# Merricx/zksnake

Measured on AMD Instinct MI355X. Metric: BN254 G1 MSM throughput, higher is better.
Workload: dtype u32 limbs (254-bit modular integers)

## Files before the change

zksnake_amd/csrc/msm_impl.hip.h:

```cpp
#pragma once
#include <algorithm>
#include <chrono>
#include <memory>
#include <vector>
#include "common.hip.h"
#include "msm_plan.h"
#include "pair.hip.h"
#include "setup_impl.hip.h"
#include "codec.hip.h"
#include "glv_params.h"

#include "msm_common.hip.h"
#include "msm_accumulate.hip.h"
#include "msm_reduce.hip.h"

namespace zkmi {
using mem::DevBuf;

#if defined(ZK_GROUP) && (!defined(ZK_PART) || ZK_PART == 0)
extern template __global__ void accumulate_kernel<ZK_GROUP>(const uint32_t*, const uint32_t*, const uint32_t*, const uint32_t*, uint32_t, uint32_t, uint32_t, uint32_t*, uint32_t*);
extern template __global__ void accumulate_split_kernel<ZK_GROUP>(const uint32_t*, const uint32_t*, const uint32_t*, const uint32_t*, uint32_t, uint32_t, uint32_t, uint32_t*, uint32_t*);
extern template __global__ void bases_to_mont_kernel<ZK_GROUP>(const uint32_t*, uint64_t, uint32_t*, int);
extern template __global__ void combine_kernel<ZK_GROUP>(const uint32_t*, const uint32_t*, uint32_t, uint32_t, const uint32_t*, const uint32_t*, uint32_t*);
extern template __global__ void strided_sum_kernel<ZK_GROUP>(const uint32_t*, uint32_t*, SumJob, SumJob, uint32_t);
extern template __global__ void weighted_sum_kernel<ZK_GROUP>(const uint32_t*, uint32_t, uint32_t, const uint32_t*, uint32_t, uint32_t*);
ZK_SETUP_EXTERN_TEMPLATES(ZK_GROUP)
ZK_CODEC_EXTERN_TEMPLATES(ZK_GROUP)
#endif

#if !defined(ZK_PART) || ZK_PART == 0

template <class G>
static int precompute_table(uint32_t* table, uint64_t n, int c, int w_first, int w_count) {
    typedef typename G::F F;
    constexpr int AW = 2 * F::LIMBS, XW = 4 * F::LIMBS;
    if (w_first == 0 && w_count == 1) return ZK_OK;
    DevBuf temp_buf;
    ZK_HIP_RC(temp_buf.alloc(n * XW * 4));
    uint32_t* const temp = temp_buf.as();
    const unsigned blocks = (unsigned)((n + 255) / 256);
    const unsigned nblocks = (unsigned)((n + (uint64_t)NORM_THREADS * NORM_E - 1) / ((uint64_t)NORM_THREADS * NORM_E));
    hipLaunchKernelGGL(dbl_rows_kernel<G>, dim3(blocks), dim3(256), 0, 0, temp, n, c * w_first, (const uint32_t*)table);
    if (w_first > 0) hipLaunchKernelGGL(normalize_kernel<G>, dim3(nblocks), dim3(NORM_THREADS), 0, 0, temp, n, table, 0);
    for (int k = 1; k < w_count; ++k) {
        hipLaunchKernelGGL(dbl_rows_kernel<G>, dim3(blocks), dim3(256), 0, 0, temp, n, c, (const uint32_t*)nullptr);
        hipLaunchKernelGGL(normalize_kernel<G>, dim3(nblocks), dim3(NORM_THREADS), 0, 0, temp, n, table + (size_t)k * n * AW, 0);
    }
    ZK_HIP(hipGetLastError());
    ZK_HIP(hipDeviceSynchronize());
    return ZK_OK;
}

template <class G>
struct FixedTable {
    std::vector<uint64_t> base;
    DevBuf d_table;
    int nwin = 0;
    std::mutex mu;
    static FixedTable& get() {
        static FixedTable* const t = new FixedTable();
        return *t;
    }
    void release() {
        std::lock_guard<std::mutex> lock(mu);
        d_table.reset();
        base.clear();
    }
    int ensure(const uint64_t* base_limbs) {
        typedef typename G::F F;
        typedef typename G::Fr FrP;
        constexpr int AW = 2 * F::LIMBS, XW = 4 * F::LIMBS;
        const size_t words64 = AW / 2;
        if (d_table && base.size() == words64 && memcmp(base.data(), base_limbs, words64 * 8) == 0) return ZK_OK;
        d_table.reset();
        base.clear();
        nwin = (FrP::BITS + 1 + FIXED_C - 1) / FIXED_C;
        std::vector<uint32_t> wb((size_t)nwin * AW);
        {
            const uint32_t* w = reinterpret_cast<const uint32_t*>(base_limbs);
            Affine<F> g = {F::from_canonical(w), F::from_canonical(w + F::LIMBS)};
            XYZZ<F> acc = xyzz_from_affine<F>(g);
            for (int j = 0; j < nwin; ++j) {
                Affine<F> a = xyzz_to_affine<F>(acc);
                F::store(wb.data() + (size_t)j * AW, a.x);
                F::store(wb.data() + (size_t)j * AW + F::LIMBS, a.y);
                if (j + 1 < nwin) for (int k = 0; k < FIXED_C; ++k) acc = xyzz_dbl<F>(acc);
            }
        }
        const uint64_t rows = (uint64_t)nwin * FIXED_HALF;
        DevBuf table, d_wb, temp;
        ZK_HIP_RC(table.alloc(rows * AW * 4));
        ZK_HIP_RC(d_wb.alloc(wb.size() * 4));
        ZK_HIP_RC(temp.alloc(rows * XW * 4));
        ZK_HIP(hipMemcpy(d_wb.as(), wb.data(), wb.size() * 4, hipMemcpyHostToDevice));
        hipLaunchKernelGGL(fixed_table_kernel<G>, dim3((unsigned)((rows + 255) / 256)), dim3(256), 0, 0, d_wb.as(), nwin, temp.as());
        hipLaunchKernelGGL(normalize_kernel<G>, dim3((unsigned)((rows + (uint64_t)NORM_THREADS * NORM_E - 1) / ((uint64_t)NORM_THREADS * NORM_E))),
                           dim3(NORM_THREADS), 0, 0, temp.as(), rows, table.as(), 0);
        ZK_HIP(hipGetLastError());
        ZK_HIP(hipDeviceSynchronize());
        d_table = std::move(table);
        base.assign(base_limbs, base_limbs + words64);
        return ZK_OK;
    }
};

template <class G>
struct MsmPlan : MsmPlanBase {
    typedef typename G::F F;
    typedef typename G::Fr FrP;
    static constexpr int AW = 2 * F::LIMBS;
    static constexpr int XW = 4 * F::LIMBS;
    static constexpr uint64_t SEG_TARGET_LANES = 256ull * 1024;
    static constexpr int MAX_C = 20;
    bool wide = false;

    struct Work {
        DevBuf partials, buckets, rows, fin;
        DevBuf parts;
        hipEvent_t ev_acc0 = nullptr, ev_accs = nullptr, ev_acc1 = nullptr;
        bool acc_from_accs = false;
        hipEvent_t ev_release = nullptr;
        bool lent = false;
        uint32_t seg_len = 0;
        int w_first = 0, w_count = 0;
        uint32_t groups = 0;
    };

    uint64_t n = 0;
    uint64_t n_api = 0;
    bool glv = false;
    bool pre = false;
    int pw_first = 0, pw_count = 0;
    uint32_t B = 0, R = 0, C = 0;
    uint32_t bpr = 0, bpc = 0;
    Work ws;
    MsmFront front;
    std::shared_ptr<DevBuf> bases_block;
    uint32_t* d_bases = nullptr;
    uint32_t* h_final = nullptr;
    hipEvent_t ev_start = nullptr, ev_end = nullptr;

    ~MsmPlan() override {
        (void)hipDeviceSynchronize();
        pinned_free_cached(h_final);
        for (hipEvent_t e : {ws.ev_acc0, ws.ev_accs, ws.ev_acc1, ws.ev_release, ev_start, ev_end}) if (e) (void)hipEventDestroy(e);
        stream_release((create_flags & ZK_MSM_HIGH_PRIORITY) != 0, own_stream);
    }

    int init(uint64_t n_points, const void* bases, int bases_on_device, int flags, int window_bits, int win_first, int win_count,
             const MsmPlan* share = nullptr) {
        const bool trace = opt.trace_init;
        auto t_prev = std::chrono::steady_clock::now();
        auto mark = [&](const char* what) {
            if (!trace) return;
            auto now = std::chrono::steady_clock::now();
            fprintf(stderr, "[plan init] %-24s %8.1f us\n", what, std::chrono::duration<double, std::micro>(now - t_prev).count());
            t_prev = now;
        };
        create_flags = flags;
        seg_lanes_at_init = opt.segment_lanes ? opt.segment_lanes : SEG_TARGET_LANES;
        pre = (flags & ZK_MSM_PRECOMPUTE) != 0;
        if (n_points == 0 || n_points > (1ull << 26)) return fail(ZK_ERR_ARG, "MSM size must be in [1, 2^26]");
        const MsmLayout lay = msm_layout(FrP::BITS, GlvOf<G>::OK, n_points, flags, window_bits, win_count <= 0);
        glv = share ? share->glv : lay.glv;
        n_api = n_points;
        n = glv ? 2 * n_points : n_points;
        entries_per_window = n;
        c = lay.c;
        if (c < 2 || c > MAX_C) return fail(ZK_ERR_ARG, "window bits must be in [2, 20]");
        if (c > 16 && !pre) return fail(ZK_ERR_ARG, "windows wider than 16 bits need a fixed-base plan (ZK_MSM_PRECOMPUTE)");
        wide = c > 16;
        nwin = glv ? glv_window_count(c) : window_count(FrP::BITS + 1, c);
        if (win_count <= 0) { win_first = 0; win_count = nwin; }
        if (win_first < 0 || win_first + win_count > nwin) return fail(ZK_ERR_ARG, "window range out of bounds");
        pw_first = win_first;
        pw_count = win_count;
        B = 1u << (c - 1);
        int rl = (c - 1 + 1) / 2;
        if (rl > 8 && !wide) rl = 8;
        R = 1u << rl;
        C = B / R;
        if (C > 1024 || R > 1024) return fail(ZK_ERR_ARG, "window too wide for the reduction stage");
        bpr = (R + WS_BLOCK - 1) / WS_BLOCK;
        bpc = (C + WS_BLOCK - 1) / WS_BLOCK;
        const uint64_t entries = (uint64_t)pw_count * n;
        if (entries > 0x7FFFFFFFull) return fail(ZK_ERR_ARG, "MSM too large");

        ZK_HIP_RC(stream_acquire((flags & ZK_MSM_HIGH_PRIORITY) != 0, &own_stream));
        if (share) {
            bases_block = share->bases_block;
            d_bases = share->d_bases;
        } else {
            bases_block = std::make_shared<DevBuf>();
            ZK_HIP_RC(bases_block->alloc((pre ? (uint64_t)pw_count : 1ull) * n * AW * 4));
            d_bases = bases_block->as();
            if (bases_on_device) {
                hipLaunchKernelGGL(bases_to_mont_kernel<G>, dim3((unsigned)((n_api + 127) / 128)), dim3(128), 0, 0,
                                   (const uint32_t*)bases, n_api, d_bases, glv ? 1 : 0);
            } else {
                DevBuf tmp;
                ZK_HIP_RC(tmp.alloc(n_api * AW * 4));
                ZK_HIP(hipMemcpy(tmp.as(), bases, n_api * AW * 4, hipMemcpyHostToDevice));
                hipLaunchKernelGGL(bases_to_mont_kernel<G>, dim3((unsigned)((n_api + 127) / 128)), dim3(128), 0, 0, tmp.as(), n_api, d_bases, glv ? 1 : 0);
                ZK_HIP(hipDeviceSynchronize());
            }
            ZK_HIP(hipGetLastError());
            if (pre) {
                int rc = precompute_table<G>(d_bases, n, c, pw_first, pw_count);
                if (rc) return rc;
            }
        }
        mark("stream + bases");
        {
            FrontLayout fl;
            fl.c = c; fl.B = B; fl.n = n; fl.n_api = n_api; fl.pre = pre; fl.wide = wide; fl.glv = glv ? &GlvOf<G>::P::K : nullptr;
            fl.pw_first = pw_first; fl.pw_count = pw_count; fl.nwin = nwin; fl.curve = G::CURVE;
            ZK_HIP_RC(front.init(fl, &opt));
        }
        const uint64_t max_sets = pre ? 1ull : (uint64_t)pw_count;
        ZK_HIP_RC(pinned_alloc_cached((void**)&h_final, (size_t)max_sets * (bpr + bpc) * 2 * XW * 4));
        mark("scalars/digits/pinned");
        ZK_HIP(hipEventCreateWithFlags(&ev_start, hipEventDisableSystemFence));
        ZK_HIP(hipEventCreate(&ev_end));
        {
            const uint64_t keys = max_sets * B;
            const uint32_t seg_full = pick_seg_len(entries);
            const uint64_t max_segs = std::max<uint64_t>(entries / seg_full, std::min<uint64_t>(entries / 8, seg_lanes_at_init)) + keys + 8;
            ZK_HIP_RC(front.alloc_workspace());
            ZK_HIP_RC(ws.partials.alloc(max_segs * XW * 4));
            ZK_HIP_RC(ws.buckets.alloc(keys * XW * 4));
            ZK_HIP_RC(ws.rows.alloc(max_sets * (R + C) * XW * 4));
            if (sum_part_len() >= 2) ZK_HIP_RC(ws.parts.alloc(max_sets * 2 * (uint64_t)(B / sum_part_len()) * XW * 4));
            ZK_HIP_RC(ws.fin.alloc(max_sets * (bpr + bpc) * 2 * XW * 4));
            for (hipEvent_t* e : {&ws.ev_acc0, &ws.ev_accs, &ws.ev_acc1, &ws.ev_release}) ZK_HIP(hipEventCreate(e));
        }
        mark("workspace + events");
        ZK_HIP_RC(front.set_kernel_attributes());
        ZK_HIP(hipFuncSetAttribute((const void*)weighted_sum_kernel<G>, hipFuncAttributeMaxDynamicSharedMemorySize,
                                   (int)(HalfRegs<F>::COUNT * HS_THREADS * 4)));
        mark("func attributes");
        ZK_HIP(hipDeviceSynchronize());
        mark("device sync");
        return ZK_OK;
    }

    uint32_t sum_part_len() const {
        const uint32_t k = 16u;
        return (R >= 4 * k && C >= 4 * k) ? k : 0u;
    }

    uint32_t pick_seg_len(uint64_t entries) const {
        const uint64_t target = opt.segment_lanes ? opt.segment_lanes : SEG_TARGET_LANES;
        uint64_t sl = (entries + target - 1) / target;
        if (sl < 8) sl = 8;
        if (sl > 64) sl = 64;
        if (pre) {
            uint64_t per_bucket = entries / B;
            uint64_t want = (per_bucket + 11) / 12;
            if (want > sl) sl = want;
            if (sl > 1024) sl = 1024;
        }
        return (uint32_t)sl;
    }


    int stage_accumulate(uint32_t m, const SortedView& sv, hipStream_t st, bool prio_steps) {
        Work& l = ws;
        uint32_t *const partials = l.partials.as(), *const buckets = l.buckets.as();
        const uint32_t seg_len = sv.seg_len;
        const uint32_t n_keys = l.groups * B;
        const uint64_t lanes_needed = ((uint64_t)l.w_count * m + seg_len - 1) / seg_len;
        bool launched = false;
        if constexpr (AccumulateSplit<G>::ON) {
            if (opt.split_pairs < 0 ? AccumulateSplit<G>::DEFAULT : opt.split_pairs != 0) {
                hipLaunchKernelGGL(accumulate_split_kernel<G>, dim3((unsigned)((2 * lanes_needed + 255) / 256)), dim3(256), 0, st, d_bases, sv.sorted, sv.bstart, sv.sstart, n_keys, seg_len, prio_steps ? 1u : 0u, partials, buckets);
                launched = true;
            }
        }
        if (!launched) hipLaunchKernelGGL(accumulate_kernel<G>, dim3((unsigned)((lanes_needed + 255) / 256)), dim3(256), 0, st, d_bases, sv.sorted, sv.bstart, sv.sstart, n_keys, seg_len, prio_steps ? 1u : 0u, partials, buckets);
        ZK_HIP(hipEventRecord(l.ev_acc1, st));
        const uint32_t small_blocks = (2 * n_keys + COMBINE_THREADS - 1) / COMBINE_THREADS;
        hipLaunchKernelGGL(combine_kernel<G>, dim3(small_blocks + COMBINE_WAVE_BLOCKS + COMBINE_BIG_BLOCKS), dim3(COMBINE_THREADS), 0, st,
                           partials, sv.sstart, n_keys, small_blocks, sv.big_list, sv.big_count, buckets);
        ZK_HIP(hipGetLastError());
        return ZK_OK;
    }

    int stage_reduce(hipStream_t st) {
        Work& l = ws;
        uint32_t *const buckets = l.buckets.as(), *const parts = l.parts.as(), *const row_sums = l.rows.as(), *const fin = l.fin.as();
        const uint32_t groups = l.groups;
        const uint32_t n_keys = groups * B;
        uint32_t n_rows = groups * R, n_cols = groups * C;
        SumJob rows = {n_rows, R, B, C, 1u, C, 0u};
        SumJob cols = {n_cols, C, B, 1u, C, R, n_rows};
        const bool one_step = opt.sum_one_step;
        const uint32_t K = (one_step || n_keys < (1u << 18)) ? 0u : sum_part_len();
        if (K >= 2 && parts && C % K == 0 && R % K == 0 && C / K >= 2 && R / K >= 2) {
            const uint32_t pr = C / K, pc = R / K;
            SumJob prow = {n_rows * pr, R * pr, B, C, 1u, K, 0u, pr, K};
            SumJob pcol = {n_cols * pc, C * pc, B, 1u, C, K, n_rows * pr, pc, K * C};
            hipLaunchKernelGGL(strided_sum_kernel<G>, dim3((unsigned)((((uint64_t)prow.n_out + pcol.n_out) * 2 + 255) / 256)), dim3(256), 0, st, buckets, parts, prow, pcol, 2u);
            SumJob frow = {n_rows, n_rows, 0u, pr, 1u, pr, 0u};
            SumJob fcol = {n_cols, n_cols, 0u, pc, 1u, pc, n_rows, 1u, 0u, n_rows * pr};
            const uint32_t lpo2 = 2 * std::min<uint32_t>(32u, std::max(pr, pc) / 2);
            hipLaunchKernelGGL(strided_sum_kernel<G>, dim3(((n_rows + n_cols) * lpo2 + 255) / 256), dim3(256), 0, st, parts, row_sums, frow, fcol, lpo2);
        } else {
        const uint32_t lpo_env = opt.lanes_per_output;
        const uint32_t lpo = lpo_env ? lpo_env : ((n_rows + n_cols) >= 4096 ? 32u : 64u);
        hipLaunchKernelGGL(strided_sum_kernel<G>, dim3(((n_rows + n_cols) * lpo + 255) / 256), dim3(256), 0, st, buckets, row_sums, rows, cols, lpo);
        }
        hipLaunchKernelGGL(weighted_sum_kernel<G>, dim3(groups * (bpr + bpc)), dim3(HS_THREADS), (size_t)HalfRegs<F>::COUNT * HS_THREADS * 4, st,
                           row_sums, R, groups, row_sums + (size_t)n_rows * XW, C, fin);
        ZK_HIP(hipGetLastError());
        ZK_HIP(hipMemcpyAsync(h_final, fin, (size_t)groups * (bpr + bpc) * 2 * XW * 4, hipMemcpyDeviceToHost, st));
        return ZK_OK;
    }

    int run_stages(uint32_t m, uint32_t dstride, hipStream_t st, const SortExport* borrowed = nullptr, int phase = 0, hipEvent_t gate = nullptr) {
        Work& l = ws;
        int rc;
        const uint32_t seg_len = borrowed ? borrowed->view.seg_len : (phase == 2 ? l.seg_len : pick_seg_len((uint64_t)l.w_count * m));
        l.seg_len = seg_len;
        if (phase == 2) {
        } else if (borrowed) {
            ZK_HIP(hipStreamWaitEvent(st, borrowed->sorted_ready, 0));
        } else if ((rc = front.sort(m, dstride, seg_len, l.w_first, l.w_count, l.groups, st))) {
            return rc;
        }
        const SortedView sv = borrowed ? borrowed->view : front.view();
        if (phase != 2) ZK_HIP(hipEventRecord(l.ev_acc0, st));
        if (phase == 1) return ZK_OK;
        if (gate) ZK_HIP(hipStreamWaitEvent(st, gate, 0));
        l.acc_from_accs = gate != nullptr || phase == 2;
        if (l.acc_from_accs) ZK_HIP(hipEventRecord(l.ev_accs, st));
        const bool prio_steps = opt.priority_steps && phase == 0 && !gate && !borrowed;
        if ((rc = stage_accumulate(m, sv, st, prio_steps))) return rc;
        if (borrowed) ZK_HIP(hipEventRecord(borrowed->release, st));
        return stage_reduce(st);
    }

    int set_option(const char* name, int64_t value) override {
        std::lock_guard<std::mutex> lock(mu);
        if (q_pending || q_sorted) return fail(ZK_ERR_ARG, "MSM plan has a run in flight: options change between runs");
        if (!strcmp(name, "segment_lanes")) {
            if (value < 64) return fail(ZK_ERR_ARG, "segment_lanes must be at least 64");
            if ((uint64_t)value > seg_lanes_at_init) return fail(ZK_ERR_ARG, "segment_lanes cannot exceed the value the plan was created with");
            opt.segment_lanes = (uint64_t)value;
        } else if (!strcmp(name, "sum_one_step")) {
            opt.sum_one_step = value != 0;
        } else if (!strcmp(name, "lanes_per_output")) {
            if (value != 0 && (value < 2 || value > 64 || (value & (value - 1)))) return fail(ZK_ERR_ARG, "lanes_per_output: 0 or a power of two in [2, 64]");
            opt.lanes_per_output = (uint32_t)value;
        } else if (!strcmp(name, "priority_steps")) {
            opt.priority_steps = value != 0;
        } else if (!strcmp(name, "split_pairs")) {
            if (value < -1 || value > 1) return fail(ZK_ERR_ARG, "split_pairs: -1 (the group's default), 0 or 1");
            if (value == 1 && !AccumulateSplit<G>::ON) return fail(ZK_ERR_ARG, "split_pairs: this group has no pair-split accumulate kernel (base-field groups)");
            opt.split_pairs = (int)value;
        } else if (!strcmp(name, "two_level_sort")) {
            if (value && !front.has_two_level_buffers()) return fail(ZK_ERR_ARG, "the plan was created without the buffers of the two-level sort");
            if (!value && wide) return fail(ZK_ERR_ARG, "windows wider than 16 bits exist in the two-level sort only");
            opt.two_level_sort = value != 0;
        } else {
            return fail(ZK_ERR_ARG, std::string("unknown or creation-time MSM option: ") + name);
        }
        return ZK_OK;
    }

    int debug_view(uint64_t* out, int cap) override {
        std::lock_guard<std::mutex> lock(mu);
        if (q_pending || q_sorted) return fail(ZK_ERR_ARG, "MSM plan has a run in flight: the view is read between runs");
        if (!out || cap < ZK_MSM_VIEW_SLOTS) return fail(ZK_ERR_ARG, "zk_msm_plan_debug_view needs room for ZK_MSM_VIEW_SLOTS values");
        bool split_acc = false;
        if constexpr (AccumulateSplit<G>::ON) split_acc = opt.split_pairs < 0 ? AccumulateSplit<G>::DEFAULT : opt.split_pairs != 0;
        const SortedView own = front.view();
        const uint64_t v[ZK_MSM_VIEW_SLOTS] = {
            (uint64_t)(uintptr_t)front.digits_buf(), (uint64_t)(uintptr_t)d_bases, (uint64_t)(uintptr_t)own.sorted, (uint64_t)(uintptr_t)own.bstart,
            (uint64_t)(uintptr_t)own.sstart, (uint64_t)(uintptr_t)own.big_list, (uint64_t)(uintptr_t)own.big_count,
            (uint64_t)(uintptr_t)ws.partials.as(), (uint64_t)(uintptr_t)ws.buckets.as(),
            n, n_api, (uint64_t)c, (uint64_t)nwin, B, glv ? 1u : 0u, pre ? 1u : 0u, wide ? 1u : 0u, (uint64_t)pw_first, (uint64_t)pw_count,
            (uint64_t)ws.w_first, (uint64_t)ws.w_count, ws.groups, ws.seg_len, q_m, front.view_dstride,
            (uint64_t)front.view_route, (uint64_t)front.view_fine_log, front.view_split_fine() ? 1u : 0u, split_acc ? 1u : 0u};
        for (int k = 0; k < ZK_MSM_VIEW_SLOTS; ++k) out[k] = v[k];
        return ZK_OK;
    }

    uint64_t seg_lanes_at_init = 0;
    int create_flags = 0;
    int clone(MsmPlanBase** out) override {
        MsmPlan* p = new MsmPlan();
        p->opt = opt;
        int rc = p->init(n_api, nullptr, 0, create_flags & ~ZK_MSM_HIGH_PRIORITY, c, pw_first, pw_count, this);
        if (rc) {
            delete p;
            return rc;
        }
        *out = p;
        return ZK_OK;
    }

    int q_first = 0, q_count = 0;
    uint32_t q_m = 0;
    hipStream_t q_stream = nullptr;
    bool q_pending = false;

    bool q_sorted = false;

    int enqueue(uint64_t n_scalars, const void* scalars, int on_device, int w_first, int w_count, hipStream_t st) override {
        return enqueue_phase(n_scalars, scalars, on_device, w_first, w_count, st, 0);
    }
    int enqueue_sort(uint64_t n_scalars, const void* scalars, int on_device, int w_first, int w_count, hipStream_t st) override {
        return enqueue_phase(n_scalars, scalars, on_device, w_first, w_count, st, 1);
    }
    hipEvent_t accumulate_done_event() override { return ws.ev_acc1; }
    int enqueue_rest(MsmPlanBase* after) override {
        std::lock_guard<std::mutex> lock(mu);
        if (!q_sorted) return fail(ZK_ERR_ARG, "zk_msm_plan_enqueue_rest without zk_msm_plan_enqueue_sort");
        q_sorted = false;
        if (q_m > 0) {
            int rc = run_stages(q_m, (q_m + 7u) & ~7u, q_stream, nullptr, 2, after ? after->accumulate_done_event() : nullptr);
            if (rc) return rc;
            ZK_HIP(hipEventRecord(ev_end, q_stream));
        }
        q_pending = true;
        return ZK_OK;
    }

    int enqueue_phase(uint64_t n_scalars, const void* scalars, int on_device, int w_first, int w_count, hipStream_t st, int phase) {
        std::lock_guard<std::mutex> lock(mu);
        if (q_pending || q_sorted) return fail(ZK_ERR_ARG, "MSM plan already has a run in flight: call zk_msm_plan_finish first");
        if (n_scalars > n_api) return fail(ZK_ERR_LENGTH, "Number of points and scalars mismatch");
        if (w_count <= 0) { w_first = pw_first; w_count = pw_count; }
        if (w_first < pw_first || w_first + w_count > pw_first + pw_count)
            return fail(ZK_ERR_ARG, "window range out of bounds (the plan was created for windows [" + std::to_string(pw_first) + ", " +
                                        std::to_string(pw_first + pw_count) + "))");
        const uint32_t m_api = (uint32_t)n_scalars;
        const uint32_t m = glv ? 2 * m_api : m_api;
        q_first = w_first; q_count = w_count; q_m = m; q_stream = st;
        if (ws.lent) {
            ZK_HIP(hipStreamWaitEvent(st, ws.ev_release, 0));
            ws.lent = false;
        }
        if (m > 0) {
            const uint32_t* sc = (const uint32_t*)scalars;
            if (!on_device) {
                ZK_HIP(hipMemcpyAsync(front.scalars_buf(), scalars, (size_t)m_api * FrP::W * 4, hipMemcpyHostToDevice, st));
                sc = front.scalars_buf();
            }
            const uint32_t dstride = (m + 7u) & ~7u;
            ZK_HIP(hipEventRecord(ev_start, st));
            int rc = front.digits(sc, m_api, w_first, w_count, st);
            if (rc) return rc;
            ws.w_first = w_first;
            ws.w_count = w_count;
            ws.groups = pre ? 1u : (uint32_t)w_count;
            if ((rc = run_stages(m, dstride, st, nullptr, phase))) return rc;
            if (phase == 0) ZK_HIP(hipEventRecord(ev_end, st));
        }
        if (phase == 1) q_sorted = true;
        else q_pending = true;
        return ZK_OK;
    }

    int cancel() override {
        std::lock_guard<std::mutex> lock(mu);
        if ((q_pending || q_sorted) && q_stream) ZK_HIP(hipStreamSynchronize(q_stream));
        q_pending = q_sorted = false;
        return ZK_OK;
    }

    int export_sort(SortExport* out) override {
        std::lock_guard<std::mutex> lock(mu);
        if ((!q_pending && !q_sorted) || q_m == 0) return fail(ZK_ERR_ARG, "the lending plan has no run in flight");
        out->view = front.view();
        out->view.seg_len = ws.seg_len;
        out->n = n; out->m = q_m; out->groups = ws.groups;
        out->c = c; out->nwin = nwin; out->w_first = q_first; out->w_count = q_count;
        out->pw_first = pw_first; out->pw_count = pw_count; out->scalar_bits = FrP::BITS; out->pre = pre; out->glv = glv;
        out->endo = glv ? G::ENDO_ID : 0;
        out->sorted_ready = ws.ev_acc0;
        out->release = ws.ev_release;
        ws.lent = true;
        return ZK_OK;
    }

    int enqueue_shared(MsmPlanBase* lender, hipStream_t st) override {
        SortExport ex;
        int rc = lender->export_sort(&ex);
        if (rc) return rc;
        std::lock_guard<std::mutex> lock(mu);
        if (q_pending || q_sorted) return fail(ZK_ERR_ARG, "MSM plan already has a run in flight: call zk_msm_plan_finish first");
        if (ex.n != n || ex.c != c || ex.nwin != nwin || ex.pre != pre || ex.glv != glv || ex.endo != (glv ? G::ENDO_ID : 0) || ex.scalar_bits != FrP::BITS ||
            ex.pw_first != pw_first || ex.pw_count != pw_count)
            return fail(ZK_ERR_ARG, "plans differ in size, window layout or mode: the sort cannot be shared");
        if (ws.lent) {
            ZK_HIP(hipStreamWaitEvent(st, ws.ev_release, 0));
            ws.lent = false;
        }
        q_first = ex.w_first; q_count = ex.w_count; q_m = ex.m; q_stream = st;
        ZK_HIP(hipEventRecord(ev_start, st));
        ws.w_first = ex.w_first;
        ws.w_count = ex.w_count;
        ws.groups = ex.groups;
        rc = run_stages(ex.m, (ex.m + 7u) & ~7u, st, &ex);
        if (rc) return rc;
        ZK_HIP(hipEventRecord(ev_end, st));
        q_pending = true;
        return ZK_OK;
    }

    int finish(uint64_t* out) override {
        std::lock_guard<std::mutex> lock(mu);
        if (q_sorted) return fail(ZK_ERR_ARG, "zk_msm_plan_finish before zk_msm_plan_enqueue_rest");
        if (!q_pending) return fail(ZK_ERR_ARG, "zk_msm_plan_finish without a pending run");
        q_pending = false;
        typedef typename G::HostF HF;
        XYZZ<HF> total = xyzz_inf<HF>();
        std::chrono::steady_clock::time_point tail_t0;
        if (q_m > 0) {
            ZK_HIP(hipEventSynchronize(ev_end));
            tail_t0 = std::chrono::steady_clock::now();
            int lc = 0;
            while ((1u << lc) < C) ++lc;
            const int groups = (int)ws.groups;
            const uint32_t* rows_fin = h_final;
            const uint32_t* cols_fin = h_final + (size_t)groups * bpr * 2 * XW;
            auto pt = [](const uint32_t* p) { return HF::xyzz_from_device(p); };
            bool first_set = true;
            for (int g = groups - 1; g >= 0; --g) {
                XYZZ<HF> sum_s = xyzz_inf<HF>(), sum_t = xyzz_inf<HF>(), x_r = xyzz_inf<HF>();
                for (int k = (int)bpr - 1; k >= 0; --k) {
                    const uint32_t* q = rows_fin + ((size_t)g * bpr + k) * 2 * XW;
                    sum_s = xyzz_add<HF>(sum_s, pt(q));
                    if (k > 0) {
                        sum_t = xyzz_add<HF>(sum_t, pt(q + XW));
                        x_r = xyzz_add<HF>(x_r, sum_t);
                    } else {
                        sum_t = xyzz_add<HF>(sum_t, pt(q + XW));
                    }
                }
                XYZZ<HF> sum_sc = xyzz_inf<HF>(), x_c = xyzz_inf<HF>(), suf_c = xyzz_inf<HF>();
                for (int k = (int)bpc - 1; k >= 0; --k) {
                    const uint32_t* q = cols_fin + ((size_t)g * bpc + k) * 2 * XW;
                    sum_sc = xyzz_add<HF>(sum_sc, pt(q));
                    if (k > 0) {
                        suf_c = xyzz_add<HF>(suf_c, pt(q + XW));
                        x_c = xyzz_add<HF>(x_c, suf_c);
                    }
                }
                int at = first_set ? -1 : c;
                auto step = [&](int exp, const XYZZ<HF>& term, bool present) {
                    if (!present) return;
                    if (at >= 0) for (int k = 0; k < at - exp; ++k) total = xyzz_dbl<HF>(total);
                    total = xyzz_add<HF>(total, term);
                    at = exp;
                };
                if (bpr > 1 && lc + WS_BLOCK_LOG > c && !first_set) return fail(ZK_ERR_ARG, "internal: reduction layout does not fit the window");
                step(lc + WS_BLOCK_LOG, x_r, bpr > 1);
                step(lc, sum_s, true);
                step(WS_BLOCK_LOG, x_c, bpc > 1);
                step(0, xyzz_add<HF>(sum_sc, sum_t), true);
                first_set = false;
            }
            if (!pre) for (int k = 0; k < c * q_first; ++k) total = xyzz_dbl<HF>(total);
            float sort_ms = 0, acc_ms = 0, red_ms = 0, t = 0;
            if (hipEventElapsedTime(&t, ev_start, ws.ev_acc0) == hipSuccess) sort_ms += t;
            if (hipEventElapsedTime(&t, ws.acc_from_accs ? ws.ev_accs : ws.ev_acc0, ws.ev_acc1) == hipSuccess) acc_ms += t;
            if (hipEventElapsedTime(&t, ws.ev_acc1, ev_end) == hipSuccess) red_ms += t;
            timings[0] = sort_ms;
            timings[1] = acc_ms;
            timings[2] = red_ms;
        }
        HF::affine_to_canonical(xyzz_to_affine<HF>(total), out);
        if (q_m > 0) {
            timings[3] = std::chrono::duration<float, std::milli>(std::chrono::steady_clock::now() - tail_t0).count();
            float t = 0;
            timings[4] = hipEventElapsedTime(&t, ev_start, ev_end) == hipSuccess ? t + timings[3] : 0.0f;
        }
        return ZK_OK;
    }
};

constexpr uint64_t FIXED_BASE_MIN = 2048;

template <class G>
static int batch_mul_impl(uint64_t n, const uint64_t* scalars, const uint64_t* bases, int broadcast, uint64_t* out) {
    typedef typename G::F F;
    typedef typename G::Fr FrP;
    constexpr int AW = 2 * F::LIMBS, XW = 4 * F::LIMBS;
    if (n == 0) return ZK_OK;
    DevBuf ds, db, dout, temp;
    const bool fixed = broadcast && n >= FIXED_BASE_MIN;
    uint64_t nb = broadcast ? 1 : n;
    ZK_HIP_RC(ds.alloc(n * FrP::W * 4));
    ZK_HIP_RC(temp.alloc(n * XW * 4));
    ZK_HIP_RC(dout.alloc(n * AW * 4));
    ZK_HIP(hipMemcpy(ds.as(), scalars, n * FrP::W * 4, hipMemcpyHostToDevice));
    if (fixed) {
        FixedTable<G>& ft = FixedTable<G>::get();
        std::lock_guard<std::mutex> lock(ft.mu);
        ZK_HIP_RC(ft.ensure(bases));
        FixedBias bias;
        memset(&bias, 0, sizeof(bias));
        for (int j = 0; j < ft.nwin; ++j) {
            int bit = j * FIXED_C + (FIXED_C - 1);
            bias.v[bit >> 5] |= 1u << (bit & 31);
        }
        hipLaunchKernelGGL(fixed_mul_kernel<G>, dim3((unsigned)((n + 255) / 256)), dim3(256), 0, 0, ds.as(), n, ft.d_table.as(), ft.nwin, bias, temp.as());
        ZK_HIP(hipDeviceSynchronize());
    } else {
        ZK_HIP_RC(db.alloc(nb * AW * 4));
        ZK_HIP(hipMemcpy(db.as(), bases, nb * AW * 4, hipMemcpyHostToDevice));
        hipLaunchKernelGGL(varbase_mul_kernel<G>, dim3((unsigned)((n + 127) / 128)), dim3(128), 0, 0, ds.as(), db.as(), broadcast, n, temp.as());
    }
    hipLaunchKernelGGL(normalize_kernel<G>, dim3((unsigned)((n + (uint64_t)NORM_THREADS * NORM_E - 1) / ((uint64_t)NORM_THREADS * NORM_E))),
                       dim3(NORM_THREADS), 0, 0, temp.as(), n, dout.as(), 1);
    ZK_HIP(hipGetLastError());
    ZK_HIP(hipMemcpy(out, dout.as(), n * AW * 4, hipMemcpyDeviceToHost));
    return ZK_OK;
}

template <class G>
static int codec_impl(uint64_t n, const void* in, void* out, int to_bytes, uint64_t* bad_index) {
    typedef typename G::F F;
    constexpr size_t ROW = (size_t)2 * F::LIMBS * 4, ENC = CodecLayout<G>::TOTAL;
    if (n == 0) return ZK_OK;
    const size_t in_bytes = n * (to_bytes ? ROW : ENC), out_bytes = n * (to_bytes ? ENC : ROW);
    DevBuf din, dout, derr;
    ZK_HIP_RC(din.alloc(in_bytes));
    ZK_HIP_RC(dout.alloc(out_bytes));
    ZK_HIP_RC(derr.alloc(8));
    unsigned long long first = ~0ull;
    ZK_HIP(hipMemcpy(din.as(), in, in_bytes, hipMemcpyHostToDevice));
    ZK_HIP(hipMemcpy(derr.as(), &first, 8, hipMemcpyHostToDevice));
    const dim3 grid((unsigned)((n + 127) / 128)), block(128);
    if (to_bytes) hipLaunchKernelGGL(points_encode_kernel<G>, grid, block, 0, 0, din.as<const uint32_t>(), n, dout.as<uint8_t>(), derr.as<unsigned long long>());
    else hipLaunchKernelGGL(points_decode_kernel<G>, grid, block, 0, 0, din.as<const uint8_t>(), n, dout.as(), derr.as<unsigned long long>());
    ZK_HIP(hipGetLastError());
    ZK_HIP(hipMemcpy(&first, derr.as(), 8, hipMemcpyDeviceToHost));
    if (first != ~0ull) {
        if (bad_index) *bad_index = (uint64_t)(first >> 8);
        return fail(ZK_ERR_POINT, codec_message((int)(first & 0xFF)));
    }
    ZK_HIP(hipMemcpy(out, dout.as(), out_bytes, hipMemcpyDeviceToHost));
    return ZK_OK;
}


#endif

}
```

zksnake_amd/csrc/msm_plan.h:

```cpp
#pragma once
#include <cstdint>
#include <cstdlib>
#include <cstring>
#include <mutex>
#include <hip/hip_runtime.h>
#include "../../include/zkmi.h"
#include "dev_buf.h"
#include "msm_front.h"

namespace zkmi {

struct SortExport {
    SortedView view;
    uint64_t n = 0;
    uint32_t m = 0, groups = 0;
    int c = 0, nwin = 0, w_first = 0, w_count = 0, pw_first = 0, pw_count = 0, scalar_bits = 0;
    bool pre = false, glv = false;
    int endo = 0;
    hipEvent_t sorted_ready = nullptr;
    hipEvent_t release = nullptr;
};

constexpr int GLV_BITS = 128;
constexpr uint64_t GLV_MAX_POINTS = 1ull << 22;
constexpr int MSM_WIDE_C_DEFAULT = 20;

inline int msm_log2(uint64_t v) {
    int l = 0;
    while (v >>= 1) ++l;
    return l;
}

inline int window_count(int bits, int c) {
    return (bits + c - 1) / c + (c == 2 ? 1 : 0);
}
inline int glv_window_count(int c) { return window_count(GLV_BITS, c); }

inline int pick_window_bits(uint64_t entries) {
    int lg = msm_log2(entries < 2 ? 2 : entries);
    int c = lg >= 16 ? 16 : lg - 2;
    if (c < 4) c = 4;
    return c;
}

struct MsmLayout {
    int c = 0, nwin = 0;
    bool glv = false;
    uint64_t entries = 0;
};

inline MsmLayout msm_layout(int scalar_bits, bool has_glv, uint64_t n_points, int flags, int window_bits, bool all_windows) {
    MsmLayout L;
    const bool pre = (flags & ZK_MSM_PRECOMPUTE) != 0;
    const bool no_glv = getenv("ZKMI_NO_GLV") != nullptr;
    L.glv = has_glv && !pre && !(flags & ZK_MSM_NO_GLV) && !no_glv && n_points <= GLV_MAX_POINTS;
    L.entries = L.glv ? 2 * n_points : n_points;
    int c = window_bits > 0 ? window_bits : pick_window_bits(L.entries);
    if (window_bits <= 0 && pre && all_windows) {
        const int pre_c = getenv("ZKMI_PRE_C") ? atoi(getenv("ZKMI_PRE_C")) : 0;
        const bool no_two_level = getenv("ZKMI_NO_TWO_LEVEL") != nullptr;
        const int cands[3] = {pre_c ? pre_c : MSM_WIDE_C_DEFAULT, 17, 0};
        for (int k = 0; !no_two_level && cands[k] > 16; ++k) {
            const int cand = cands[k];
            const uint64_t w = (uint64_t)(scalar_bits + 1 + cand - 1) / cand;
            const int top_bits = scalar_bits + 1 - (int)(w - 1) * cand;
            if (n_points >= (1ull << 20) && w < 16 && (2 * top_bits >= cand || pre_c) && w * n_points <= 0x7FFFFFFFull) { c = cand; break; }
            if (pre_c) break;
        }
    }
    L.c = c;
    L.nwin = c > 0 ? (L.glv ? glv_window_count(c) : window_count(scalar_bits + 1, c)) : 0;
    return L;
}

struct MsmOptions {
    uint64_t segment_lanes = 256ull * 1024;
    bool sum_one_step = false;
    uint32_t lanes_per_output = 0;
    bool two_level_sort = true;
    bool priority_steps = true;
    int split_pairs = -1;
    uint32_t sort_workgroups = 256;
    int fine_log = 0;
    bool trace_init = false;

    static MsmOptions from_env() {
        MsmOptions o;
        if (const char* e = getenv("ZKMI_SEG_LANES")) o.segment_lanes = (uint64_t)atoll(e);
        o.sum_one_step = getenv("ZKMI_SUM_ONE_STEP") != nullptr;
        if (const char* e = getenv("ZKMI_LPO")) o.lanes_per_output = (uint32_t)atoi(e);
        o.two_level_sort = getenv("ZKMI_NO_TWO_LEVEL") == nullptr;
        o.priority_steps = getenv("ZKMI_NO_PRIO_STEPS") == nullptr;
        if (const char* e = getenv("ZKMI_SPLIT_PAIRS")) o.split_pairs = atoi(e) != 0 ? 1 : 0;
        if (const char* e = getenv("ZKMI_SORT_WGS")) o.sort_workgroups = (uint32_t)atoi(e);
        if (const char* e = getenv("ZKMI_FINE_LOG")) o.fine_log = atoi(e);
        o.trace_init = getenv("ZKMI_TRACE_INIT") != nullptr;
        return o;
    }
};

struct MsmPlanBase {
    virtual ~MsmPlanBase() {}
    MsmOptions opt = MsmOptions::from_env();
    virtual int set_option(const char* name, int64_t value) = 0;
    virtual int export_sort(SortExport* out) = 0;
    virtual int debug_view(uint64_t* out, int cap) = 0;
    virtual int enqueue_shared(MsmPlanBase* lender, hipStream_t stream) = 0;
    virtual int clone(MsmPlanBase** out) = 0;
    virtual int enqueue(uint64_t n_scalars, const void* scalars, int on_device, int w_first, int w_count,
                        hipStream_t stream) = 0;
    virtual int enqueue_sort(uint64_t n_scalars, const void* scalars, int on_device, int w_first, int w_count, hipStream_t stream) = 0;
    virtual int enqueue_rest(MsmPlanBase* after) = 0;
    virtual hipEvent_t accumulate_done_event() = 0;
    virtual int finish(uint64_t* out) = 0;
    virtual int cancel() = 0;
    int run(uint64_t n_scalars, const void* scalars, int on_device, int w_first, int w_count, uint64_t* out,
            hipStream_t stream) {
        int rc = enqueue(n_scalars, scalars, on_device, w_first, w_count, stream);
        return rc ? rc : finish(out);
    }
    hipStream_t own_stream = nullptr;
    int c = 0, nwin = 0;
    uint64_t entries_per_window = 0;
    float timings[5] = {0, 0, 0, 0, 0};
    std::mutex mu;
};


#define ZK_DECLARE_GROUP(G)                                                                                              \
    int msm_plan_create_##G(uint64_t n, const void* bases, int on_device, int flags, int window_bits, int window_first,    \
                            int window_count, MsmPlanBase** out);                                                        \
    int msm_batch_mul_##G(uint64_t n, const uint64_t* scalars, const uint64_t* bases, int broadcast, uint64_t* out);     \
    int msm_points_codec_##G(uint64_t n, const void* in, void* out, int to_bytes, uint64_t* bad_index);                  \
    void msm_fixed_table_free_##G();
ZK_DECLARE_GROUP(Bn254G1)
ZK_DECLARE_GROUP(Bn254G2)
ZK_DECLARE_GROUP(Bls381G1)
ZK_DECLARE_GROUP(Bls381G2)
#undef ZK_DECLARE_GROUP

}
```

zksnake_amd/csrc/msm_reduce.hip.h:

```cpp
#pragma once
#include "msm_common.hip.h"

namespace zkmi {

constexpr int COMBINE_THREADS = 256;
constexpr uint32_t COMBINE_WAVE_BLOCKS = 128, COMBINE_BIG_BLOCKS = 64;

template <class G>
__global__ __launch_bounds__(COMBINE_THREADS) void combine_kernel(const uint32_t* __restrict__ partials,
                                                                  const uint32_t* __restrict__ run_start, uint32_t n_keys,
                                                                  uint32_t small_blocks, const uint32_t* __restrict__ big_list,
                                                                  const uint32_t* __restrict__ big_count,
                                                                  uint32_t* __restrict__ buckets) {
    typedef typename G::F F;
    constexpr int XW = 4 * F::LIMBS;
    constexpr int HW = HalfRegs<F>::COUNT;
    __shared__ uint32_t sh[COMBINE_THREADS * HW];
    const bool odd = (threadIdx.x & 1) != 0;
    if (blockIdx.x < small_blocks) {
        const uint32_t key = (blockIdx.x * COMBINE_THREADS + threadIdx.x) >> 1;
        if (key >= n_keys) return;
        const uint32_t s0 = run_start[key], s1 = run_start[key + 1];
        if (s1 - s0 == 1 || s1 - s0 > COMBINE_SMALL_MAX) return;
        HalfPt<F> acc = half_inf<F>();
        if (s1 > s0) {
            acc = half_load<F>(partials + (size_t)s0 * XW, odd);
            HalfPt<F> cur = s0 + 1 < s1 ? half_load<F>(partials + (size_t)(s0 + 1) * XW, odd) : half_inf<F>();
            for (uint32_t r = s0 + 1; r < s1; ++r) {
                HalfPt<F> nxt = r + 1 < s1 ? half_load<F>(partials + (size_t)(r + 1) * XW, odd) : half_inf<F>();
                acc = pair_add<F>(acc, cur, odd);
                cur = nxt;
            }
        }
        half_store<F>(buckets + (size_t)key * XW, odd, acc);
    } else if (blockIdx.x < small_blocks + COMBINE_WAVE_BLOCKS) {
        const uint32_t count = big_count[0];
        const uint32_t lane = threadIdx.x & 63, pair = lane >> 1;
        const uint32_t wave = ((blockIdx.x - small_blocks) * COMBINE_THREADS + threadIdx.x) >> 6;
        const uint32_t n_waves = (COMBINE_WAVE_BLOCKS * COMBINE_THREADS) >> 6;
        for (uint32_t b = wave; b < count; b += n_waves) {
            const uint32_t key = big_list[b];
            const uint32_t s0 = run_start[key], s1 = run_start[key + 1];
            HalfPt<F> v = half_inf<F>();
            for (uint32_t r = s0 + pair; r < s1; r += 32) v = pair_add<F>(v, half_load<F>(partials + (size_t)r * XW, odd), odd);
            for (int m = 32; m >= 2; m >>= 1) v = pair_add<F>(v, half_shfl_xor<F>(v, m), odd);
            if (lane < 2) half_store<F>(buckets + (size_t)key * XW, odd, v);
        }
    } else {
        const uint32_t count = big_count[1];
        const uint32_t j = threadIdx.x, pair = j >> 1;
        for (uint32_t b = blockIdx.x - small_blocks - COMBINE_WAVE_BLOCKS; b < count; b += COMBINE_BIG_BLOCKS) {
            const uint32_t key = big_list[n_keys - 1 - b];
            const uint32_t s0 = run_start[key], s1 = run_start[key + 1];
            HalfPt<F> v = half_inf<F>();
            for (uint32_t r = s0 + pair; r < s1; r += COMBINE_THREADS / 2) v = pair_add<F>(v, half_load<F>(partials + (size_t)r * XW, odd), odd);
            for (uint32_t off = COMBINE_THREADS / 4; off >= 1; off >>= 1) {
                half_lds_put<F>(sh, COMBINE_THREADS, j, v);
                __syncthreads();
                if (pair < off) v = pair_add<F>(v, half_lds_get<F>(sh, COMBINE_THREADS, j + 2 * off), odd);
                __syncthreads();
            }
            if (j < 2) half_store<F>(buckets + (size_t)key * XW, odd, v);
        }
    }
}


struct SumJob {
    uint32_t n_out, per_group, group_stride, outer, inner, count;
    uint32_t out_offset;
    uint32_t split = 1, outer2 = 0;
    uint32_t in_offset = 0;
};

template <class G>
__global__ __launch_bounds__(256) void strided_sum_kernel(const uint32_t* __restrict__ in, uint32_t* __restrict__ out,
                                                          SumJob j0, SumJob j1, uint32_t lpo) {
    typedef typename G::F F;
    constexpr int XW = 4 * F::LIMBS;
    const uint32_t gid = blockIdx.x * blockDim.x + threadIdx.x;
    uint32_t o = gid / lpo;
    const uint32_t sub = gid % lpo;
    const bool odd = (sub & 1) != 0;
    const uint32_t pair = sub >> 1, n_pairs = lpo >> 1;
    SumJob job = j0;
    if (o >= j0.n_out) {
        o -= j0.n_out;
        job = j1;
    }
    const bool live = o < job.n_out;
    const uint32_t x = live ? o % job.per_group : 0;
    size_t base = live ? (size_t)job.in_offset + (size_t)(o / job.per_group) * job.group_stride + (size_t)(x / job.split) * job.outer + (size_t)(x % job.split) * job.outer2 : 0;
    HalfPt<F> acc = half_inf<F>();
    if (live && pair < job.count) {
        HalfPt<F> cur = half_load<F>(in + (base + (size_t)pair * job.inner) * XW, odd);
        for (uint32_t j = pair; j < job.count; j += n_pairs) {
            const uint32_t jn = j + n_pairs < job.count ? j + n_pairs : j;
            HalfPt<F> nxt = half_load<F>(in + (base + (size_t)jn * job.inner) * XW, odd);
            acc = pair_add<F>(acc, cur, odd);
            cur = nxt;
        }
    }
    for (uint32_t m = lpo >> 1; m >= 2; m >>= 1) {
        HalfPt<F> other = half_shfl_xor<F>(acc, (int)m);
        acc = pair_add<F>(acc, other, odd);
    }
    if (live && sub < 2) half_store<F>(out + ((size_t)job.out_offset + o) * XW, odd, acc);
}

constexpr int WS_BLOCK = 128;
constexpr int WS_BLOCK_LOG = 7;
constexpr int HS_THREADS = 2 * WS_BLOCK;
template <class G>
__global__ __launch_bounds__(HS_THREADS) void weighted_sum_kernel(const uint32_t* __restrict__ in0, uint32_t m0, uint32_t n0,
                                                                  const uint32_t* __restrict__ in1, uint32_t m1,
                                                                  uint32_t* __restrict__ out) {
    typedef typename G::F F;
    constexpr int XW = 4 * F::LIMBS;
    extern __shared__ uint32_t sh[];
    const uint32_t tid = threadIdx.x, pj = tid >> 1;
    const bool odd = (tid & 1) != 0;
    const uint32_t bpa0 = (m0 + WS_BLOCK - 1) / WS_BLOCK, bpa1 = (m1 + WS_BLOCK - 1) / WS_BLOCK;
    const bool first = blockIdx.x < n0 * bpa0;
    const uint32_t rel = first ? blockIdx.x : blockIdx.x - n0 * bpa0;
    const uint32_t bpa = first ? bpa0 : bpa1, ma = first ? m0 : m1;
    const uint32_t arr_i = rel / bpa, blk = rel % bpa;
    const uint32_t m = min((uint32_t)WS_BLOCK, ma - blk * WS_BLOCK);
    const uint32_t* arr = (first ? in0 : in1) + ((size_t)arr_i * ma + (size_t)blk * WS_BLOCK) * XW;
    HalfPt<F> v = pj < m ? half_load<F>(arr + (size_t)pj * XW, odd) : half_inf<F>();
    for (uint32_t off = 1; off < m; off <<= 1) {
        half_lds_put<F>(sh, HS_THREADS, tid, v);
        __syncthreads();
        if (pj + off < m) {
            HalfPt<F> o = half_lds_get<F>(sh, HS_THREADS, tid + 2 * off);
            v = pair_add<F>(v, o, odd);
        }
        __syncthreads();
    }
    if (pj == 0) half_store<F>(out + ((size_t)blockIdx.x * 2 + 1) * XW, odd, v);
    if (pj == 0 || pj >= m) v = half_inf<F>();
    uint32_t top = 1;
    while (top < m) top <<= 1;
    for (uint32_t off = top / 2; off >= 1; off >>= 1) {
        half_lds_put<F>(sh, HS_THREADS, tid, v);
        __syncthreads();
        if (pj < off) {
            HalfPt<F> o = half_lds_get<F>(sh, HS_THREADS, tid + 2 * off);
            v = pair_add<F>(v, o, odd);
        }
        __syncthreads();
    }
    if (pj == 0) half_store<F>(out + (size_t)blockIdx.x * 2 * XW, odd, v);
}

}
```

Measured before the change: 693.1.

## Pack leftover combine runs into a shared queue and write final sums to mapped host memory

The combine kernel's small-key path now adds the first two partials for every key in one pass. Keys with more than two runs are pushed to a shared-memory queue, and the block's lanes then work through that queue together, which evens out the divergent per-key serial loops within a wave. The weighted sum kernel also writes its result straight into pinned, device-mapped host memory, removing the separate device buffer and the device-to-host memcpy. Results are then written over the bus from device stores, so correctness now relies on stream sync covering visibility of those zero-copy writes. The packed path is the default and can be switched off through a new option.

```diff
diff --git a/zksnake_amd/csrc/msm_impl.hip.h b/zksnake_amd/csrc/msm_impl.hip.h
--- a/zksnake_amd/csrc/msm_impl.hip.h
+++ b/zksnake_amd/csrc/msm_impl.hip.h
@@ -115,7 +115,7 @@
     bool wide = false;
 
     struct Work {
-        DevBuf partials, buckets, rows, fin;
+        DevBuf partials, buckets, rows;
         DevBuf parts;
         hipEvent_t ev_acc0 = nullptr, ev_accs = nullptr, ev_acc1 = nullptr;
         bool acc_from_accs = false;
@@ -138,6 +138,7 @@
     std::shared_ptr<DevBuf> bases_block;
     uint32_t* d_bases = nullptr;
     uint32_t* h_final = nullptr;
+    uint32_t* d_final = nullptr;
     hipEvent_t ev_start = nullptr, ev_end = nullptr;
 
     ~MsmPlan() override {
@@ -219,6 +220,7 @@
         }
         const uint64_t max_sets = pre ? 1ull : (uint64_t)pw_count;
         ZK_HIP_RC(pinned_alloc_cached((void**)&h_final, (size_t)max_sets * (bpr + bpc) * 2 * XW * 4));
+        ZK_HIP(hipHostGetDevicePointer((void**)&d_final, h_final, 0));
         mark("scalars/digits/pinned");
         ZK_HIP(hipEventCreateWithFlags(&ev_start, hipEventDisableSystemFence));
         ZK_HIP(hipEventCreate(&ev_end));
@@ -231,7 +233,6 @@
             ZK_HIP_RC(ws.buckets.alloc(keys * XW * 4));
             ZK_HIP_RC(ws.rows.alloc(max_sets * (R + C) * XW * 4));
             if (sum_part_len() >= 2) ZK_HIP_RC(ws.parts.alloc(max_sets * 2 * (uint64_t)(B / sum_part_len()) * XW * 4));
-            ZK_HIP_RC(ws.fin.alloc(max_sets * (bpr + bpc) * 2 * XW * 4));
             for (hipEvent_t* e : {&ws.ev_acc0, &ws.ev_accs, &ws.ev_acc1, &ws.ev_release}) ZK_HIP(hipEventCreate(e));
         }
         mark("workspace + events");
@@ -281,14 +282,14 @@
         ZK_HIP(hipEventRecord(l.ev_acc1, st));
         const uint32_t small_blocks = (2 * n_keys + COMBINE_THREADS - 1) / COMBINE_THREADS;
         hipLaunchKernelGGL(combine_kernel<G>, dim3(small_blocks + COMBINE_WAVE_BLOCKS + COMBINE_BIG_BLOCKS), dim3(COMBINE_THREADS), 0, st,
-                           partials, sv.sstart, n_keys, small_blocks, sv.big_list, sv.big_count, buckets);
+                           partials, sv.sstart, n_keys, small_blocks | (opt.combine_packed == 0 ? COMBINE_UNPACKED : 0u), sv.big_list, sv.big_count, buckets);
         ZK_HIP(hipGetLastError());
         return ZK_OK;
     }
 
     int stage_reduce(hipStream_t st) {
         Work& l = ws;
-        uint32_t *const buckets = l.buckets.as(), *const parts = l.parts.as(), *const row_sums = l.rows.as(), *const fin = l.fin.as();
+        uint32_t *const buckets = l.buckets.as(), *const parts = l.parts.as(), *const row_sums = l.rows.as();
         const uint32_t groups = l.groups;
         const uint32_t n_keys = groups * B;
         uint32_t n_rows = groups * R, n_cols = groups * C;
@@ -311,9 +312,8 @@
         hipLaunchKernelGGL(strided_sum_kernel<G>, dim3(((n_rows + n_cols) * lpo + 255) / 256), dim3(256), 0, st, buckets, row_sums, rows, cols, lpo);
         }
         hipLaunchKernelGGL(weighted_sum_kernel<G>, dim3(groups * (bpr + bpc)), dim3(HS_THREADS), (size_t)HalfRegs<F>::COUNT * HS_THREADS * 4, st,
-                           row_sums, R, groups, row_sums + (size_t)n_rows * XW, C, fin);
+                           row_sums, R, groups, row_sums + (size_t)n_rows * XW, C, d_final);
         ZK_HIP(hipGetLastError());
-        ZK_HIP(hipMemcpyAsync(h_final, fin, (size_t)groups * (bpr + bpc) * 2 * XW * 4, hipMemcpyDeviceToHost, st));
         return ZK_OK;
     }
 
@@ -358,6 +358,9 @@
             if (value < -1 || value > 1) return fail(ZK_ERR_ARG, "split_pairs: -1 (the group's default), 0 or 1");
             if (value == 1 && !AccumulateSplit<G>::ON) return fail(ZK_ERR_ARG, "split_pairs: this group has no pair-split accumulate kernel (base-field groups)");
             opt.split_pairs = (int)value;
+        } else if (!strcmp(name, "combine_packed")) {
+            if (value < -1 || value > 1) return fail(ZK_ERR_ARG, "combine_packed: -1 (the default), 0 or 1");
+            opt.combine_packed = (int)value;
         } else if (!strcmp(name, "two_level_sort")) {
             if (value && !front.has_two_level_buffers()) return fail(ZK_ERR_ARG, "the plan was created without the buffers of the two-level sort");
             if (!value && wide) return fail(ZK_ERR_ARG, "windows wider than 16 bits exist in the two-level sort only");
diff --git a/zksnake_amd/csrc/msm_plan.h b/zksnake_amd/csrc/msm_plan.h
--- a/zksnake_amd/csrc/msm_plan.h
+++ b/zksnake_amd/csrc/msm_plan.h
@@ -80,6 +80,7 @@
     bool two_level_sort = true;
     bool priority_steps = true;
     int split_pairs = -1;
+    int combine_packed = -1;
     uint32_t sort_workgroups = 256;
     int fine_log = 0;
     bool trace_init = false;
@@ -92,6 +93,7 @@
         o.two_level_sort = getenv("ZKMI_NO_TWO_LEVEL") == nullptr;
         o.priority_steps = getenv("ZKMI_NO_PRIO_STEPS") == nullptr;
         if (const char* e = getenv("ZKMI_SPLIT_PAIRS")) o.split_pairs = atoi(e) != 0 ? 1 : 0;
+        if (const char* e = getenv("ZKMI_COMBINE_PACKED")) o.combine_packed = atoi(e) != 0 ? 1 : 0;
         if (const char* e = getenv("ZKMI_SORT_WGS")) o.sort_workgroups = (uint32_t)atoi(e);
         if (const char* e = getenv("ZKMI_FINE_LOG")) o.fine_log = atoi(e);
         o.trace_init = getenv("ZKMI_TRACE_INIT") != nullptr;
diff --git a/zksnake_amd/csrc/msm_reduce.hip.h b/zksnake_amd/csrc/msm_reduce.hip.h
--- a/zksnake_amd/csrc/msm_reduce.hip.h
+++ b/zksnake_amd/csrc/msm_reduce.hip.h
@@ -5,19 +5,57 @@
 
 constexpr int COMBINE_THREADS = 256;
 constexpr uint32_t COMBINE_WAVE_BLOCKS = 128, COMBINE_BIG_BLOCKS = 64;
+constexpr uint32_t COMBINE_UNPACKED = 1u << 31;
+constexpr uint32_t COMBINE_QUEUE_WORDS = 1 + 3 * (COMBINE_THREADS / 2);
+
+__host__ __device__ constexpr uint32_t combine_queue_at(uint32_t slot, uint32_t field) { return 1u + 3u * slot + field; }
 
 template <class G>
 __global__ __launch_bounds__(COMBINE_THREADS) void combine_kernel(const uint32_t* __restrict__ partials,
                                                                   const uint32_t* __restrict__ run_start, uint32_t n_keys,
-                                                                  uint32_t small_blocks, const uint32_t* __restrict__ big_list,
+                                                                  uint32_t small_blocks_flags, const uint32_t* __restrict__ big_list,
                                                                   const uint32_t* __restrict__ big_count,
                                                                   uint32_t* __restrict__ buckets) {
     typedef typename G::F F;
     constexpr int XW = 4 * F::LIMBS;
     constexpr int HW = HalfRegs<F>::COUNT;
     __shared__ uint32_t sh[COMBINE_THREADS * HW];
+    static_assert(COMBINE_QUEUE_WORDS <= (uint32_t)COMBINE_THREADS * HW, "the leftover queue lives in the tree's staging array");
+    const uint32_t small_blocks = small_blocks_flags & ~COMBINE_UNPACKED;
     const bool odd = (threadIdx.x & 1) != 0;
-    if (blockIdx.x < small_blocks) {
+    if (blockIdx.x < small_blocks && !(small_blocks_flags & COMBINE_UNPACKED)) {
+        const uint32_t key = (blockIdx.x * COMBINE_THREADS + threadIdx.x) >> 1;
+        const bool live = key < n_keys;
+        const uint32_t s0 = live ? run_start[key] : 0u, s1 = live ? run_start[key + 1] : 0u;
+        const uint32_t runs = s1 - s0;
+        const bool mine = live && runs != 1 && runs <= COMBINE_SMALL_MAX;
+        if (threadIdx.x == 0) sh[0] = 0;
+        __syncthreads();
+        if (mine) {
+            HalfPt<F> acc = half_inf<F>();
+            if (runs >= 2) acc = pair_add<F>(half_load<F>(partials + (size_t)s0 * XW, odd), half_load<F>(partials + (size_t)(s0 + 1) * XW, odd), odd);
+            half_store<F>(buckets + (size_t)key * XW, odd, acc);
+            if (runs > 2 && !odd) {
+                const uint32_t slot = atomicAdd(&sh[0], 1u);
+                sh[combine_queue_at(slot, 0)] = key;
+                sh[combine_queue_at(slot, 1)] = s0 + 2;
+                sh[combine_queue_at(slot, 2)] = s1;
+            }
+        }
+        __syncthreads();
+        const uint32_t e = threadIdx.x >> 1;
+        if (e < sh[0]) {
+            const uint32_t k2 = sh[combine_queue_at(e, 0)], r0 = sh[combine_queue_at(e, 1)], r1 = sh[combine_queue_at(e, 2)];
+            HalfPt<F> acc = half_load<F>(buckets + (size_t)k2 * XW, odd);
+            HalfPt<F> cur = half_load<F>(partials + (size_t)r0 * XW, odd);
+            for (uint32_t r = r0; r < r1; ++r) {
+                HalfPt<F> nxt = r + 1 < r1 ? half_load<F>(partials + (size_t)(r + 1) * XW, odd) : half_inf<F>();
+                acc = pair_add<F>(acc, cur, odd);
+                cur = nxt;
+            }
+            half_store<F>(buckets + (size_t)k2 * XW, odd, acc);
+        }
+    } else if (blockIdx.x < small_blocks) {
         const uint32_t key = (blockIdx.x * COMBINE_THREADS + threadIdx.x) >> 1;
         if (key >= n_keys) return;
         const uint32_t s0 = run_start[key], s1 = run_start[key + 1];
```

Result: no change. 692.4 (-0.1%).
